# xmindflow/TransCeption

Hardware: AMD Instinct MI355X
Metric: images/sec fwd+bwd at 224x224 B=16 per GPU (higher is better)
Workload: dtype bf16; 1 GPU; TransCeption (MSTransception) 224x224 B=16/GPU fwd+bwd+SGD, synthetic Synapse npz slices via the device loader, name-seeded random-init weights; global_batch=16, image_size=224, parallelism=dp1, headline_mode=loader, headline_degraded=False, launch_mode=hipGraph replay

## Files before the change

transception_amd/build.py:

```python
from __future__ import annotations

import concurrent.futures as cf
import os
import subprocess
import sys

HERE = os.path.dirname(os.path.abspath(__file__))
CSRC = os.path.join(HERE, "csrc")
LIB = os.path.join(HERE, "libtransception_hip.so")
SOURCES = ["gemm.hip", "norm.hip", "dwconv.hip", "softmax.hip", "attention.hip", "attention_seg.hip", "elementwise.hip", "train.hip", "factoratt.hip", "data.hip", "mixffn.hip", "mixffn_bwd.hip", "effatt.hip", "cbam.hip", "ripm.hip", "linln.hip", "lncls.hip", "legacy.hip", "metrics.hip"]
FLAGS = ["--offload-arch=gfx950", "-O3", "-std=c++17", "-fPIC", "-ffp-contract=fast", "-munsafe-fp-atomics"]


def _hipcc() -> str:
    for c in (os.environ.get("HIPCC"), "/opt/rocm/bin/hipcc", "hipcc"):
        if c and (os.path.isabs(c) and os.path.exists(c) or not os.path.isabs(c)):
            return c
    raise RuntimeError("hipcc not found")


def _stale(target: str, deps) -> bool:
    if not os.path.exists(target):
        return True
    t = os.path.getmtime(target)
    return any(os.path.getmtime(d) > t for d in deps)


def build(force: bool = False, verbose: bool = True) -> str:
    hipcc = _hipcc()
    genv = {k: v for k, v in os.environ.items() if not k.startswith(("TC_ATTN_", "TC_AS_", "TC_DKV_", "TC_DQ_"))}
    for gen in ("gen_attn_asm.py", "gen_dkv_asm.py", "gen_dq_asm.py"):
        r = subprocess.run([sys.executable, os.path.join(CSRC, gen)], capture_output=True, text=True, env=genv)
        if r.returncode != 0:
            raise RuntimeError(f"{gen} failed:\n{r.stderr}")
    headers = [os.path.join(CSRC, "tc_common.h"), os.path.join(HERE, "..", "include", "transception_hip.h")]
    extra = {"attention_seg.hip": [os.path.join(CSRC, "attn_fwd_asm.inc"), os.path.join(CSRC, "attn_dkv_asm.inc"), os.path.join(CSRC, "attn_dq_asm.inc")]}
    objdir = os.path.join(HERE, "build")
    os.makedirs(objdir, exist_ok=True)
    jobs = []
    for src in SOURCES:
        s = os.path.join(CSRC, src)
        o = os.path.join(objdir, src.replace(".hip", ".o"))
        if force or _stale(o, [s] + headers + extra.get(src, [])):
            jobs.append((s, o))

    extra_flags = {"lncls.hip": ["-fno-slp-vectorize"]}

    def compile_one(job):
        s, o = job
        cmd = [hipcc, *FLAGS, *extra_flags.get(os.path.basename(s), []), "-c", s, "-o", o]
        r = subprocess.run(cmd, capture_output=True, text=True)
        if r.returncode != 0:
            raise RuntimeError(f"hipcc failed for {s}:\n{r.stderr}")
        return s

    with cf.ThreadPoolExecutor(max_workers=min(6, max(1, len(jobs)))) as ex:
        for s in ex.map(compile_one, jobs):
            if verbose:
                print(f"[build] compiled {os.path.basename(s)}")
    objs = [os.path.join(objdir, s.replace(".hip", ".o")) for s in SOURCES]
    if force or jobs or _stale(LIB, objs):
        r = subprocess.run([hipcc, "--offload-arch=gfx950", "-shared", "-fPIC", "-o", LIB, *objs], capture_output=True, text=True)
        if r.returncode != 0:
            raise RuntimeError(f"link failed:\n{r.stderr}")
        if verbose:
            print(f"[build] linked {LIB}")
    return LIB


if __name__ == "__main__":
    build(force="--force" in sys.argv)
```

transception_amd/csrc/effatt.hip:

```cpp
#include "tc_common.h"
#include <cstdlib>

namespace {

typedef float f32x16 __attribute__((ext_vector_type(16)));
typedef short s16x4_t __attribute__((ext_vector_type(4)));
typedef short s16x8_t __attribute__((ext_vector_type(8)));

constexpr int C = 64, PT = C + 8, TPW = 256, NW = 4, RT = 32 * NW, NRD = TPW / RT;
constexpr int TOUT = RT;
constexpr int F_M = 0, F_S = C, F_P = 2 * C, F_N = 2 * C + C * C;
constexpr int B1_DCTX = 0, B1_DWR = C * C, B1_DWQ = 2 * C * C, B1_DBR = 3 * C * C, B1_DBQ = B1_DBR + C, B1_N = B1_DBQ + C;
constexpr int B2_DWK = 0, B2_DWV = C * C, B2_DBK = 2 * C * C, B2_DBV = B2_DBK + C, B2_DG = B2_DBV + C, B2_DB = B2_DG + C, B2_N = B2_DB + C;
constexpr int SCW = 64 * 33;

struct EffDev {
    const void* t; const void* gamma; const void* beta;
    const void* wk; const void* bk; const void* wq; const void* bq; const void* wv; const void* bv; const void* wr; const void* br;
    void* out; float* ctx; float* kstat; float* part; float* dctx; float* rsum;
    const void* dout; void* dt; void* g1;
    int ldt, ldo, lddo, lddt, acc_dt, B, N, wpi;
    float eps;
};

template <typename V8> __device__ __forceinline__ V8 ld_tr(const bf16_t* lo, const bf16_t* hi) {
    const s16x4_t a = __builtin_amdgcn_ds_read_tr16_b64_v4i16((s16x4_t __attribute__((address_space(3)))*)(lo));
    const s16x4_t b = __builtin_amdgcn_ds_read_tr16_b64_v4i16((s16x4_t __attribute__((address_space(3)))*)(hi));
    return __builtin_bit_cast(V8, (s16x8_t)__builtin_shufflevector(a, b, 0, 1, 2, 3, 4, 5, 6, 7));
}
template <typename H> __device__ __forceinline__ void up8s(const uint4& r, float* o) {
    unpack2<H>(r.x, o[0], o[1]); unpack2<H>(r.y, o[2], o[3]); unpack2<H>(r.z, o[4], o[5]); unpack2<H>(r.w, o[6], o[7]);
}
struct Lane { int lane, l31, hh, gi, gq2, wv; };
__device__ __forceinline__ Lane lane_of() {
    Lane L; L.lane = threadIdx.x & 63; L.wv = threadIdx.x >> 6; L.l31 = L.lane & 31; L.hh = L.lane >> 5; L.gi = L.lane & 15; L.gq2 = (L.lane >> 4) & 1;
    return L;
}

__device__ __forceinline__ void zero2(f32x16 (&a)[2]) {
#pragma unroll
    for (int cb = 0; cb < 2; ++cb)
#pragma unroll
        for (int r = 0; r < 16; ++r) a[cb][r] = 0.f;
}
template <typename H> __device__ __forceinline__ void mm_w(const bf16_t* W, const bf16_t* X, const Lane& L, f32x16 (&acc)[2]) {
    using V8 = typename TcHalf<H>::v8;
#pragma unroll
    for (int kk = 0; kk < C / 16; ++kk) {
        const V8 xv = *reinterpret_cast<const V8*>(X + L.l31 * PT + kk * 16 + 8 * L.hh);
#pragma unroll
        for (int cb = 0; cb < 2; ++cb) acc[cb] = TcHalf<H>::mfma(*reinterpret_cast<const V8*>(W + (cb * 32 + L.l31) * PT + kk * 16 + 8 * L.hh), xv, acc[cb]);
    }
}
// ... 630 lines not shown
    if (!bwd) return f->out && !(f->ldo & 7) && !((uintptr_t)f->out & 15);
    if (!f->dout || !f->dt || !f->g1 || (f->lddo & 7) || (f->lddt & 7) || ((uintptr_t)f->dout & 15) || ((uintptr_t)f->dt & 15) || ((uintptr_t)f->g1 & 15)) return false;
    return f->dgamma && f->dbeta && f->dwk && f->dbk && f->dwq && f->dbq && f->dwv && f->dbv && f->dwr && f->dbr;
}
long long eff_scratch(int B, int N) {
    const long long nwv = (long long)B * ((N + TPW - 1) / TPW);
    const long long per = (B1_N + B2_N) > F_N ? (B1_N + B2_N) : F_N;
    return nwv * per + (long long)B * C * C + (long long)B * C;
}
EffDev eff_dev(const TcEffAtt* f) {
    EffDev p;
    p.t = f->t; p.gamma = f->gamma; p.beta = f->beta; p.wk = f->wk; p.bk = f->bk; p.wq = f->wq; p.bq = f->bq; p.wv = f->wv; p.bv = f->bv; p.wr = f->wr; p.br = f->br;
    p.out = f->out; p.ctx = f->ctx; p.kstat = f->kstat; p.part = f->part; p.dout = f->dout; p.dt = f->dt; p.g1 = f->g1;
    p.ldt = f->ldt; p.ldo = f->ldo; p.lddo = f->lddo; p.lddt = f->lddt; p.acc_dt = f->acc_dt; p.B = f->B; p.N = f->N; p.eps = f->eps;
    p.wpi = (f->N + TPW - 1) / TPW;
    const long long nwv = (long long)f->B * p.wpi;
    const long long per = (B1_N + B2_N) > F_N ? (B1_N + B2_N) : F_N;
    p.dctx = f->part + nwv * per;
    p.rsum = p.dctx + (long long)f->B * C * C;
    return p;
}

template <typename H> int eff_fwd(const TcEffAtt* f, hipStream_t s) {
    const EffDev p = eff_dev(f);
    const int nwv = f->B * p.wpi;
    hipLaunchKernelGGL((effatt_kv_kernel<H>), dim3(nwv), dim3(64 * NW), 0, s, p);
    if (tc_launch_status() != TC_OK) return TC_ERR_LAUNCH;
    hipLaunchKernelGGL(effatt_ctx_kernel, dim3(f->B, C), dim3(64), 0, s, p);
    if (tc_launch_status() != TC_OK) return TC_ERR_LAUNCH;
    hipLaunchKernelGGL((effatt_out_kernel<H>), dim3(f->B * ((f->N + TOUT - 1) / TOUT)), dim3(64 * NW), 0, s, p);
    return tc_launch_status();
}
template <typename H> int eff_bwd(const TcEffAtt* f, hipStream_t s) {
    const EffDev p = eff_dev(f);
    const int nwv = f->B * p.wpi;
    hipLaunchKernelGGL((effatt_bq_kernel<H>), dim3(nwv), dim3(64 * NW), 0, s, p);
    if (tc_launch_status() != TC_OK) return TC_ERR_LAUNCH;
    hipLaunchKernelGGL(effatt_dctx_kernel, dim3(f->B, C), dim3(64), 0, s, p);
    if (tc_launch_status() != TC_OK) return TC_ERR_LAUNCH;
    hipLaunchKernelGGL((effatt_bkv_kernel<H>), dim3(nwv), dim3(64 * NW), 0, s, p);
    if (tc_launch_status() != TC_OK) return TC_ERR_LAUNCH;
    FoldDev r;
    r.part = f->part; r.nwv = nwv; r.nper = B1_N + B2_N;
    float* dsts[12] = {nullptr, f->dwr, f->dwq, f->dbr, f->dbq, f->dwk, f->dwv, f->dbk, f->dbv, f->dgamma, f->dbeta, nullptr};
    const int offs[13] = {B1_DCTX, B1_DWR, B1_DWQ, B1_DBR, B1_DBQ, B1_N + B2_DWK, B1_N + B2_DWV, B1_N + B2_DBK, B1_N + B2_DBV, B1_N + B2_DG, B1_N + B2_DB, B1_N + B2_N, B1_N + B2_N};
    for (int i = 0; i < 12; ++i) r.dst[i] = dsts[i];
    for (int i = 0; i < 13; ++i) r.off[i] = offs[i];
    hipLaunchKernelGGL(effatt_fold_kernel, dim3((r.nper / 4 + 15) / 16), dim3(256), 0, s, r);
    return tc_launch_status();
}

}

extern "C" int tc_effatt_supported(int Cc, int dtype) { return Cc == C && (dtype == TC_BF16 || dtype == TC_F16); }
extern "C" long long tc_effatt_scratch_floats(int Cc, int B, int N) { return (Cc == C && B > 0 && N > 0) ? eff_scratch(B, N) : 0; }
extern "C" int tc_effatt_fwd(const TcEffAtt* f, int dtype, void* stream) {
    if (!eff_ok(f, false) || !tc_effatt_supported(f->C, dtype) || f->part_floats < eff_scratch(f->B, f->N)) return TC_ERR_ARG;
    return dtype == TC_BF16 ? eff_fwd<bf16_t>(f, (hipStream_t)stream) : eff_fwd<f16_t>(f, (hipStream_t)stream);
}
extern "C" int tc_effatt_bwd(const TcEffAtt* f, int dtype, void* stream) {
    if (!eff_ok(f, true) || !tc_effatt_supported(f->C, dtype) || f->part_floats < eff_scratch(f->B, f->N)) return TC_ERR_ARG;
    return dtype == TC_BF16 ? eff_bwd<bf16_t>(f, (hipStream_t)stream) : eff_bwd<f16_t>(f, (hipStream_t)stream);
}
```

transception_amd/engine.py:

```python
from __future__ import annotations

import ctypes as C
import os
from typing import Callable, Dict, List, Optional, Tuple

import torch

from ._lib import (ATTN_DKV_SPLITS, EW_COPY, EW_DEINTERLEAVE, EW_PATCHIFY, TcEffAtt, TcEwSeg, TcFfnBwd, TcFfnFused, ACT_COORD, ACT_GELU, ACT_HSWISH, ACT_NONE, ACT_SCALE, ACT_SIGMOID, FFN_EP, FFN_LN_A, FFN_LN_B, TC_BF16, TC_F16, TC_F32, TcDwFold, TcDwSeg, TcFfnSeg,
                   TcGemm, lib)

_DT = {torch.float32: TC_F32, torch.bfloat16: TC_BF16, torch.float16: TC_F16}

PROFILE: Optional[dict] = None


SEG_MARKS = os.environ.get("TC_SEG_MARKS", "")
SEG_LABELS: List[str] = []


def _timed(name: str, flops: float, fn):
    if PROFILE is None:
        fn()
        return
    e0, e1 = torch.cuda.Event(enable_timing=True), torch.cuda.Event(enable_timing=True)
# ... 790 lines not shown
                                   acc=1, splitk=self._splitk(t["C4"], t["Cin"], t["M"]), c_f32=1, nb1=Gn, sA=(t["M"] * t["C4"], 0),
                                   sB=(t["M"] * x.ld, 0), sC=(gs, 0), rowsum=_ptr(t["b1"].grad) if t["b1"].grad is not None else None, srow=gs,
                                   use_ws=False))
            self._launch_gemms(g2)
            for t in st:
                for k in ("gp", "part2", "dh"):
                    t.pop(k, None)
        self._rec(bwd)
        return [t["out"] for t in st_all]

    def _pass_grad_batched(self, v: Var, src: torch.Tensor, nb: int, M: int, N: int, sb_src: int, sb_dst: Optional[int] = None,
                           defer: bool = False):
        sb_dst = sb_src if sb_dst is None else sb_dst
        g, acc = self.wgrad(v, 0 if v.rows >= nb * M else (nb - 1) * sb_dst // v.root.cols)
        if defer:
            return TcEwSeg(EW_COPY, acc, src.data_ptr(), g.data_ptr(), sb_src, sb_dst, src.stride(0), g.stride(0), nb, M, N, 0, 0, 0)
        self.L.tc_copy3d(_ptr(src), sb_src, src.stride(0), _ptr(g), sb_dst, g.stride(0), nb, M, N, acc, self.dt, self.stream)

    def effatt_supported(self, t: Var, params: Optional[Tuple[P, ...]] = None) -> bool:
        if self.record and (not t.requires_grad or (params is not None and any(p.grad is None for p in params))):
            return False
        return (_EFFATT_FUSED and self.ngroups == 1 and self.dt != TC_F32
                and bool(self.L.tc_effatt_supported(t.cols, self.dt)) and t.data.is_contiguous())

    def eff_attention_block(self, t: Var, ln: Tuple[P, P], keys: Tuple[P, P], queries: Tuple[P, P], values: Tuple[P, P],
                            reproj: Tuple[P, P], B: int, N: int, eps: float = 1e-5) -> Var:
        L, Cc = self.L, t.cols
        assert t.rows == B * N and self.effatt_supported(t)
        out = self.new(t.rows, Cc)
        nf = int(L.tc_effatt_scratch_floats(Cc, B, N))
        ctx, kstat = self.f32(B, Cc, Cc), self.f32(B, 2, Cc)
        es = t.data.element_size()

        def desc(part, dout=None, dt=None, g1=None, acc=0, grads=False):
            f = TcEffAtt()
            f.t, f.gamma, f.beta = _ptr(t.data), _ptr(ln[0].data), _ptr(ln[1].data)
            for nm, (W, b) in (("k", keys), ("q", queries), ("v", values), ("r", reproj)):
                setattr(f, "w" + nm, _ptr(W.data)); setattr(f, "b" + nm, _ptr(b.data))
                if grads:
                    setattr(f, "dw" + nm, _ptr(W.grad)); setattr(f, "db" + nm, _ptr(b.grad))
            if grads:
                f.dgamma, f.dbeta = _ptr(ln[0].grad), _ptr(ln[1].grad)
            f.out, f.ctx, f.kstat, f.part, f.part_floats = _ptr(out.data), _ptr(ctx), _ptr(kstat), _ptr(part), nf
            f.ldt, f.ldo, f.C, f.B, f.N, f.eps = t.ld, out.ld, Cc, B, N, eps
            if dout is not None:
                f.dout, f.lddo, f.dt, f.lddt, f.g1, f.acc_dt = _ptr(dout), dout.stride(0), _ptr(dt), dt.stride(0), _ptr(g1), acc
            return f

        part = self.f32(nf)
        f = desc(part)
        self.n_launch += 3
        _timed("hbm:effatt_fwd (LayerNorm + EfficientAttention + residual: token statistics, context fold, output)",
               3.0 * t.rows * Cc * es, lambda: L.tc_effatt_fwd(C.byref(f), self.dt, self.stream))
        del part

        def bwd():
            dy = self.grad_of(out)
            if dy is None or not t.requires_grad:
                return
            gx, acc = self.wgrad(t)
            part = self.f32(nf)
            g1 = _empty((t.rows, Cc), self.dtype, self.dev)
            fb = desc(part, dy, gx, g1, acc, grads=True)
            self.n_launch += 4
            _timed("hbm:effatt_bwd (query side + d_ctx partials, d_ctx fold, key/value side + LayerNorm backward, parameter fold)",
                   (6.0 + acc) * t.rows * Cc * es, lambda: L.tc_effatt_bwd(C.byref(fb), self.dt, self.stream))
        self._rec(bwd)
        return out

    def layernorm(self, x: Var, g: P, b: P, eps: float = 1e-5, act: int = ACT_NONE, out: Optional[Var] = None,
                  stats: Optional[Tuple[torch.Tensor, torch.Tensor]] = None, launch: bool = True) -> Var:
        Gn = self.ngroups
        rows, Cc = x.rows // Gn, x.cols
        assert Gn == 1 or (g.gs > 0 and b.gs == g.gs)
        if out is None:
            out = self.new(x.rows, Cc)
        mean, rstd = stats if stats is not None else (self.f32(x.rows), self.f32(x.rows))
        es = x.data.element_size()
        if launch:
            _timed("hbm:layernorm_fwd", 2.0 * x.rows * Cc * es, lambda: self.L.tc_layernorm_fwd(
                _ptr(x.data), x.ld, _ptr(g.data), _ptr(b.data), _ptr(out.data), out.ld, _ptr(mean), _ptr(rstd), rows, Cc, eps, act, Gn, g.gs,
                self.dt, self.stream))

        def bwd():
            dy = self.grad_of(out)
            if dy is None or not x.requires_grad:
                return
            gx, acc = self.wgrad(x)
            fused = g.grad is not None
            nblk = int(self.L.tc_layernorm_bwd_nblk(rows, Cc)) if (fused and _LN_DEFER) else 0
            if nblk > 0:
                nf = Gn * nblk * 2 * Cc
                part = self.f32(nf)
                _timed("hbm:layernorm_bwd", (3.0 + acc) * x.rows * Cc * es, lambda: self.L.tc_layernorm_bwd_defer(
                    _ptr(dy), dy.stride(0), _ptr(x.data), x.ld, _ptr(g.data), _ptr(b.data), _ptr(mean), _ptr(rstd), _ptr(gx), gx.stride(0),
                    _ptr(gx) if acc else None, gx.stride(0), _ptr(g.grad), _ptr(b.grad), rows, Cc, act, Gn, g.gs, _ptr(part), nf, self.dt,
                    self.stream))
                self._ln_pending.append((part, g.grad, b.grad, g.gs, nblk, Cc, Gn))
                if len(self._ln_pending) == 64:
                    self._flush_param_folds()
                return
            if fused:
                ws = _workspace(self.dev)
                scratch, n = ws, ws.numel() // 4
                _timed("hbm:layernorm_bwd", (3.0 + acc) * x.rows * Cc * es, lambda: self.L.tc_layernorm_bwd(
                    _ptr(dy), dy.stride(0), _ptr(x.data), x.ld, _ptr(g.data), _ptr(b.data), _ptr(mean), _ptr(rstd), _ptr(gx), gx.stride(0),
                    _ptr(gx) if acc else None, gx.stride(0), _ptr(g.grad), _ptr(b.grad), rows, Cc, act, Gn, g.gs, _ptr(scratch), n, self.dt,
                    self.stream))
                return
            self.L.tc_layernorm_bwd(_ptr(dy), dy.stride(0), _ptr(x.data), x.ld, _ptr(g.data), _ptr(b.data), _ptr(mean),
                                    _ptr(rstd), _ptr(gx), gx.stride(0), _ptr(gx) if acc else None, gx.stride(0),
                                    None, None, rows, Cc, act, Gn, g.gs, None, 0, self.dt, self.stream)
        self._rec(bwd)
        return out
# ... 969 lines not shown
```

Measured before the change: 1463 images/sec.

## Add fused wide-channel EfficientAttention kernels for C=128 and C=320

Adds a new fused EfficientAttention path for channel widths 128 and 320. It uses three MFMA-based kernels for the forward pass (LayerNorm plus K/Q/V projections and token stats, context build, output) and a mix of fused kernels and grouped GEMMs for the backward pass. Before this, only C=64 had a fused path, so wider stages likely fell back to a sequence of generic ops. The forward now keeps its scratch buffer alive so the backward can reuse the saved intermediates (normalized input, k/q/v maps). The cost is more memory held between forward and backward, plus new code that could carry numerical or correctness risk.

```diff
diff --git a/transception_amd/build.py b/transception_amd/build.py
--- a/transception_amd/build.py
+++ b/transception_amd/build.py
@@ -8,7 +8,7 @@
 HERE = os.path.dirname(os.path.abspath(__file__))
 CSRC = os.path.join(HERE, "csrc")
 LIB = os.path.join(HERE, "libtransception_hip.so")
-SOURCES = ["gemm.hip", "norm.hip", "dwconv.hip", "softmax.hip", "attention.hip", "attention_seg.hip", "elementwise.hip", "train.hip", "factoratt.hip", "data.hip", "mixffn.hip", "mixffn_bwd.hip", "effatt.hip", "cbam.hip", "ripm.hip", "linln.hip", "lncls.hip", "legacy.hip", "metrics.hip"]
+SOURCES = ["gemm.hip", "norm.hip", "dwconv.hip", "softmax.hip", "attention.hip", "attention_seg.hip", "elementwise.hip", "train.hip", "factoratt.hip", "data.hip", "mixffn.hip", "mixffn_bwd.hip", "effatt.hip", "effatt_wide.hip", "cbam.hip", "ripm.hip", "linln.hip", "lncls.hip", "legacy.hip", "metrics.hip"]
 FLAGS = ["--offload-arch=gfx950", "-O3", "-std=c++17", "-fPIC", "-ffp-contract=fast", "-munsafe-fp-atomics"]
 
 
@@ -33,7 +33,7 @@
         r = subprocess.run([sys.executable, os.path.join(CSRC, gen)], capture_output=True, text=True, env=genv)
         if r.returncode != 0:
             raise RuntimeError(f"{gen} failed:\n{r.stderr}")
-    headers = [os.path.join(CSRC, "tc_common.h"), os.path.join(HERE, "..", "include", "transception_hip.h")]
+    headers = [os.path.join(CSRC, "tc_common.h"), os.path.join(CSRC, "effatt_wide.h"), os.path.join(HERE, "..", "include", "transception_hip.h")]
     extra = {"attention_seg.hip": [os.path.join(CSRC, "attn_fwd_asm.inc"), os.path.join(CSRC, "attn_dkv_asm.inc"), os.path.join(CSRC, "attn_dq_asm.inc")]}
     objdir = os.path.join(HERE, "build")
     os.makedirs(objdir, exist_ok=True)
diff --git a/transception_amd/csrc/effatt.hip b/transception_amd/csrc/effatt.hip
--- a/transception_amd/csrc/effatt.hip
+++ b/transception_amd/csrc/effatt.hip
@@ -1,4 +1,5 @@
 #include "tc_common.h"
+#include "effatt_wide.h"
 #include <cstdlib>
 
 namespace {
@@ -735,13 +736,18 @@
 
 }
 
-extern "C" int tc_effatt_supported(int Cc, int dtype) { return Cc == C && (dtype == TC_BF16 || dtype == TC_F16); }
-extern "C" long long tc_effatt_scratch_floats(int Cc, int B, int N) { return (Cc == C && B > 0 && N > 0) ? eff_scratch(B, N) : 0; }
+extern "C" int tc_effatt_supported(int Cc, int dtype) { return (Cc == C && (dtype == TC_BF16 || dtype == TC_F16)) || tcw::effatt_wide_supported(Cc, dtype); }
+extern "C" long long tc_effatt_scratch_floats(int Cc, int B, int N) {
+    if (Cc != C) return tcw::effatt_wide_scratch(Cc, B, N);
+    return (B > 0 && N > 0) ? eff_scratch(B, N) : 0;
+}
 extern "C" int tc_effatt_fwd(const TcEffAtt* f, int dtype, void* stream) {
+    if (f && f->C != C) return tcw::effatt_wide_fwd(f, dtype, stream);
     if (!eff_ok(f, false) || !tc_effatt_supported(f->C, dtype) || f->part_floats < eff_scratch(f->B, f->N)) return TC_ERR_ARG;
     return dtype == TC_BF16 ? eff_fwd<bf16_t>(f, (hipStream_t)stream) : eff_fwd<f16_t>(f, (hipStream_t)stream);
 }
 extern "C" int tc_effatt_bwd(const TcEffAtt* f, int dtype, void* stream) {
+    if (f && f->C != C) return tcw::effatt_wide_bwd(f, dtype, stream);
     if (!eff_ok(f, true) || !tc_effatt_supported(f->C, dtype) || f->part_floats < eff_scratch(f->B, f->N)) return TC_ERR_ARG;
     return dtype == TC_BF16 ? eff_bwd<bf16_t>(f, (hipStream_t)stream) : eff_bwd<f16_t>(f, (hipStream_t)stream);
 }
diff --git a/transception_amd/csrc/effatt_wide.h b/transception_amd/csrc/effatt_wide.h
--- /dev/null
+++ b/transception_amd/csrc/effatt_wide.h
@@ -0,0 +1,9 @@
+#pragma once
+#include "../../include/transception_hip.h"
+
+namespace tcw {
+__attribute__((visibility("hidden"))) int effatt_wide_supported(int C, int dtype);
+__attribute__((visibility("hidden"))) long long effatt_wide_scratch(int C, int B, int N);
+__attribute__((visibility("hidden"))) int effatt_wide_fwd(const TcEffAtt* f, int dtype, void* stream);
+__attribute__((visibility("hidden"))) int effatt_wide_bwd(const TcEffAtt* f, int dtype, void* stream);
+}
diff --git a/transception_amd/csrc/effatt_wide.hip b/transception_amd/csrc/effatt_wide.hip
--- /dev/null
+++ b/transception_amd/csrc/effatt_wide.hip
@@ -0,0 +1,632 @@
+#include "tc_common.h"
+#include "effatt_wide.h"
+
+namespace {
+
+typedef float f32x16 __attribute__((ext_vector_type(16)));
+typedef short s16x4_t __attribute__((ext_vector_type(4)));
+typedef short s16x8_t __attribute__((ext_vector_type(8)));
+
+constexpr int NW = 4, NT = 64 * NW, TT = 32;
+
+struct WideDev {
+    const void* t; const void* gamma; const void* beta;
+    const void* wk; const void* bk; const void* wq; const void* bq; const void* wv; const void* bv; const void* wr; const void* br;
+    void* out; float* ctx; float* kstat; const void* dout; void* dt;
+    float* dgamma; float* dbeta;
+    void* n1; void* km; void* qm; void* vm; void* am; void* dam; void* dkqv; void* ctx16;
+    float* tstat; float* dctx;
+    int ldt, ldo, lddo, lddt, acc_dt, B, N, tpi;
+    float eps;
+};
+
+template <typename V8> __device__ __forceinline__ V8 ld_tr(const bf16_t* lo, const bf16_t* hi) {
+    const s16x4_t a = __builtin_amdgcn_ds_read_tr16_b64_v4i16((s16x4_t __attribute__((address_space(3)))*)(lo));
+    const s16x4_t b = __builtin_amdgcn_ds_read_tr16_b64_v4i16((s16x4_t __attribute__((address_space(3)))*)(hi));
+    return __builtin_bit_cast(V8, (s16x8_t)__builtin_shufflevector(a, b, 0, 1, 2, 3, 4, 5, 6, 7));
+}
+template <typename H> __device__ __forceinline__ void up8(const uint4& r, float* o) {
+    unpack2<H>(r.x, o[0], o[1]); unpack2<H>(r.y, o[2], o[3]); unpack2<H>(r.z, o[4], o[5]); unpack2<H>(r.w, o[6], o[7]);
+}
+template <typename H> __device__ __forceinline__ uint4 pk8(const float* o) {
+    return make_uint4(pack2<H>(o[0], o[1]), pack2<H>(o[2], o[3]), pack2<H>(o[4], o[5]), pack2<H>(o[6], o[7]));
+}
+__device__ __forceinline__ void ldf8(const float* p, float* o) {
+    const float4 a = *reinterpret_cast<const float4*>(p), b = *reinterpret_cast<const float4*>(p + 4);
+    o[0] = a.x; o[1] = a.y; o[2] = a.z; o[3] = a.w; o[4] = b.x; o[5] = b.y; o[6] = b.z; o[7] = b.w;
+}
+template <typename H, typename WT> __device__ __forceinline__ uint4 ld8w(const WT* p) {
+    if constexpr (std::is_same<WT, float>::value) { float v[8]; ldf8(p, v); return pk8<H>(v); }
+    else return *reinterpret_cast<const uint4*>(p);
+}
+
+struct Lane { int lane, l31, hh, gi, gq2, wv; };
+__device__ __forceinline__ Lane lane_of() {
+    Lane L; L.lane = threadIdx.x & 63; L.wv = threadIdx.x >> 6; L.l31 = L.lane & 31; L.hh = L.lane >> 5; L.gi = L.lane & 15; L.gq2 = (L.lane >> 4) & 1;
+    return L;
+}
+
+template <int C, int SW> struct Geo {
+    static constexpr int PT = C + 8, PF = C + 4, PS = SW + 8;
+    static constexpr int SLAB = (SW * PT > C * PS) ? SW * PT : C * PS;
+};
+
+constexpr int slab_w(int C) { return C > 128 ? 64 : 128; }
+
+template <typename H, typename WT, int C, int SW, bool TR, bool ACC>
+__device__ __forceinline__ void tile_mm(const WT* __restrict__ W, const bf16_t* X, float* ft, bf16_t* slab, const Lane& L) {
+    using V8 = typename TcHalf<H>::v8;
+    using G = Geo<C, SW>;
+    constexpr int KSTEPS = SW == 128 ? C / 16 : C / 32;
+    const int blk = SW == 128 ? L.wv : (L.wv & 1), kh = SW == 128 ? 0 : (L.wv >> 1);
+    for (int o0 = 0; o0 < C; o0 += SW) {
+        const int nw = (C - o0) < SW ? (C - o0) : SW;
+        if (!TR) {
+            for (int i = threadIdx.x; i < nw * (C / 8); i += NT) {
+                const int r = i / (C / 8), cg = i - r * (C / 8);
+                *reinterpret_cast<uint4*>(slab + r * G::PT + cg * 8) = ld8w<H, WT>(W + (long long)(o0 + r) * C + cg * 8);
+            }
+        } else {
+            const int cpr = nw / 8;
+            for (int i = threadIdx.x; i < C * cpr; i += NT) {
+                const int r = i / cpr, cg = i - r * cpr;
+                *reinterpret_cast<uint4*>(slab + r * G::PS + cg * 8) = ld8w<H, WT>(W + (long long)r * C + o0 + cg * 8);
+            }
+        }
+        __syncthreads();
+        const bool act = blk * 32 < nw;
+        f32x16 acc;
+#pragma unroll
+        for (int r = 0; r < 16; ++r) acc[r] = 0.f;
+        if (act) {
+#pragma unroll 4
+            for (int ks = 0; ks < KSTEPS; ++ks) {
+                const int kk = kh * KSTEPS + ks;
+                const V8 xv = *reinterpret_cast<const V8*>(X + L.l31 * G::PT + kk * 16 + 8 * L.hh);
+                V8 a;
+                if (!TR) a = *reinterpret_cast<const V8*>(slab + (blk * 32 + L.l31) * G::PT + kk * 16 + 8 * L.hh);
+                else {
+                    const bf16_t* wp = slab + (16 * kk + 8 * L.hh + (L.gi >> 2)) * G::PS + blk * 32 + 16 * L.gq2 + 4 * (L.gi & 3);
+                    a = ld_tr<V8>(wp, wp + 4 * G::PS);
+                }
+                acc = TcHalf<H>::mfma(a, xv, acc);
+            }
+        }
+        float* fp = ft + L.l31 * G::PF + o0 + blk * 32 + 4 * L.hh;
+        if (SW == 128) {
+            if (act) {
+#pragma unroll
+                for (int gq = 0; gq < 4; ++gq) {
+                    float4 v = make_float4(acc[4 * gq], acc[4 * gq + 1], acc[4 * gq + 2], acc[4 * gq + 3]);
+                    if (ACC) { const float4 o = *reinterpret_cast<const float4*>(fp + 8 * gq); v.x += o.x; v.y += o.y; v.z += o.z; v.w += o.w; }
+                    *reinterpret_cast<float4*>(fp + 8 * gq) = v;
+                }
+            }
+        } else {
+#pragma unroll
+            for (int ph = 0; ph < 2; ++ph) {
+                if (act && kh == ph) {
+#pragma unroll
+                    for (int gq = 0; gq < 4; ++gq) {
+                        float4 v = make_float4(acc[4 * gq], acc[4 * gq + 1], acc[4 * gq + 2], acc[4 * gq + 3]);
+                        if (ACC || ph) { const float4 o = *reinterpret_cast<const float4*>(fp + 8 * gq); v.x += o.x; v.y += o.y; v.z += o.z; v.w += o.w; }
+                        *reinterpret_cast<float4*>(fp + 8 * gq) = v;
+                    }
+                }
+                if (ph == 0) __syncthreads();
+            }
+        }
+        __syncthreads();
+    }
+}
+
+template <typename H, int C> __device__ __forceinline__ void tile_load(bf16_t* X, const H* src, long long row0, int ld, int nv) {
+    for (int i = threadIdx.x; i < TT * (C / 8); i += NT) {
+        const int r = i / (C / 8), cg = i - r * (C / 8);
+        *reinterpret_cast<uint4*>(X + r * (C + 8) + cg * 8) = r < nv ? *reinterpret_cast<const uint4*>(src + (row0 + r) * ld + cg * 8) : make_uint4(0u, 0u, 0u, 0u);
+    }
+}
+template <typename H, int C> __device__ __forceinline__ void tile_store(const bf16_t* X, H* dst, long long row0, int ld, int nv) {
+    for (int i = threadIdx.x; i < TT * (C / 8); i += NT) {
+        const int r = i / (C / 8), cg = i - r * (C / 8);
+        if (r < nv) *reinterpret_cast<uint4*>(dst + (row0 + r) * ld + cg * 8) = *reinterpret_cast<const uint4*>(X + r * (C + 8) + cg * 8);
+    }
+}
+template <typename H, int C> __device__ __forceinline__ void load_vec(float* v, const void* src) {
+    for (int i = threadIdx.x; i < C; i += NT) v[i] = ldf<H>(reinterpret_cast<const H*>(src) + i);
+}
+template <typename H, int C> __device__ __forceinline__ void row_stats(const bf16_t* X, int r, int q, float eps, float& mean, float& rstd) {
+    float s = 0.f;
+#pragma unroll
+    for (int j = 0; j < C / 64; ++j) {
+        float v[8];
+        up8<H>(*reinterpret_cast<const uint4*>(X + r * (C + 8) + (q + 8 * j) * 8), v);
+#pragma unroll
+        for (int e = 0; e < 8; ++e) s += v[e];
+    }
+    mean = tc_group_sum<8>(s) * (1.0f / C);
+    float q2 = 0.f;
+#pragma unroll
+    for (int j = 0; j < C / 64; ++j) {
+        float v[8];
+        up8<H>(*reinterpret_cast<const uint4*>(X + r * (C + 8) + (q + 8 * j) * 8), v);
+#pragma unroll
+        for (int e = 0; e < 8; ++e) { const float d = v[e] - mean; q2 += d * d; }
+    }
+    rstd = rsqrtf(tc_group_sum<8>(q2) * (1.0f / C) + eps);
+}
+
+struct Where { int b, w; long long row0; int nv; };
+__device__ __forceinline__ Where where_am_i(int tpi, int N) {
+    Where q;
+    q.b = blockIdx.x / tpi; q.w = blockIdx.x - q.b * tpi;
+    q.row0 = (long long)q.b * N + (long long)q.w * TT;
+    q.nv = min(TT, N - q.w * TT);
+    return q;
+}
+
+template <typename H, int C>
+__global__ __launch_bounds__(NT) void wide_kqv_kernel(const WideDev p) {
+    using G = Geo<C, slab_w(C)>;
+    constexpr int PT = G::PT, PF = G::PF;
+    __shared__ __attribute__((aligned(16))) bf16_t xt[TT * PT], yt[TT * PT], slab[G::SLAB];
+    __shared__ __attribute__((aligned(16))) float ft[TT * PF];
+    __shared__ float gam[C], bet[C], bia[C];
+    const Lane L = lane_of();
+    const Where w = where_am_i(p.tpi, p.N);
+    const int r = threadIdx.x >> 3, q = threadIdx.x & 7;
+    tile_load<H, C>(xt, reinterpret_cast<const H*>(p.t), w.row0, p.ldt, w.nv);
+    load_vec<H, C>(gam, p.gamma); load_vec<H, C>(bet, p.beta); load_vec<H, C>(bia, p.bk);
+    __syncthreads();
+    {
+        float mean, rstd;
+        row_stats<H, C>(xt, r, q, p.eps, mean, rstd);
+#pragma unroll
+        for (int j = 0; j < C / 64; ++j) {
+            const int c0 = (q + 8 * j) * 8;
+            float v[8];
+            up8<H>(*reinterpret_cast<const uint4*>(xt + r * PT + c0), v);
+#pragma unroll
+            for (int e = 0; e < 8; ++e) v[e] = (v[e] - mean) * rstd * gam[c0 + e] + bet[c0 + e];
+            *reinterpret_cast<uint4*>(xt + r * PT + c0) = pk8<H>(v);
+        }
+    }
+    __syncthreads();
+    tile_store<H, C>(xt, reinterpret_cast<H*>(p.n1), w.row0, C, w.nv);
+    tile_mm<H, H, C, slab_w(C), false, false>(reinterpret_cast<const H*>(p.wk), xt, ft, slab, L);
+#pragma unroll
+    for (int j = 0; j < C / 64; ++j) {
+        const int c0 = (q + 8 * j) * 8;
+        float v[8];
+        ldf8(ft + r * PF + c0, v);
+#pragma unroll
+        for (int e = 0; e < 8; ++e) v[e] += bia[c0 + e];
+        *reinterpret_cast<uint4*>(yt + r * PT + c0) = pk8<H>(v);
+    }
+    __syncthreads();
+    tile_store<H, C>(yt, reinterpret_cast<H*>(p.km), w.row0, C, w.nv);
+    for (int c = threadIdx.x; c < C; c += NT) {
+        float m = -3.0e38f;
+        for (int rr = 0; rr < w.nv; ++rr) m = fmaxf(m, ldf<H>(reinterpret_cast<const H*>(yt) + rr * PT + c));
+        float s = 0.f;
+        for (int rr = 0; rr < w.nv; ++rr) s += __expf(ldf<H>(reinterpret_cast<const H*>(yt) + rr * PT + c) - m);
+        float* ts = p.tstat + (long long)blockIdx.x * 2 * C;
+        ts[c] = m; ts[C + c] = s;
+    }
+    __syncthreads();
+    load_vec<H, C>(bia, p.bq);
+    tile_mm<H, H, C, slab_w(C), false, false>(reinterpret_cast<const H*>(p.wq), xt, ft, slab, L);
+    {
+        float v[C / 64][8], m = -3.0e38f, s = 0.f;
+#pragma unroll
+        for (int j = 0; j < C / 64; ++j) {
+            const int c0 = (q + 8 * j) * 8;
+            ldf8(ft + r * PF + c0, v[j]);
+#pragma unroll
+            for (int e = 0; e < 8; ++e) { v[j][e] += bia[c0 + e]; m = fmaxf(m, v[j][e]); }
+        }
+        m = tc_group_max<8>(m);
+#pragma unroll
+        for (int j = 0; j < C / 64; ++j)
+#pragma unroll
+            for (int e = 0; e < 8; ++e) { v[j][e] = __expf(v[j][e] - m); s += v[j][e]; }
+        const float inv = 1.0f / tc_group_sum<8>(s);
+#pragma unroll
+        for (int j = 0; j < C / 64; ++j) {
+#pragma unroll
+            for (int e = 0; e < 8; ++e) v[j][e] *= inv;
+            *reinterpret_cast<uint4*>(yt + r * PT + (q + 8 * j) * 8) = pk8<H>(v[j]);
+        }
+    }
+    __syncthreads();
+    tile_store<H, C>(yt, reinterpret_cast<H*>(p.qm), w.row0, C, w.nv);
+    load_vec<H, C>(bia, p.bv);
+    tile_mm<H, H, C, slab_w(C), false, false>(reinterpret_cast<const H*>(p.wv), xt, ft, slab, L);
+#pragma unroll
+    for (int j = 0; j < C / 64; ++j) {
+        const int c0 = (q + 8 * j) * 8;
+        float v[8];
+        ldf8(ft + r * PF + c0, v);
+#pragma unroll
+        for (int e = 0; e < 8; ++e) v[e] += bia[c0 + e];
+        if (r < w.nv) *reinterpret_cast<uint4*>(reinterpret_cast<H*>(p.vm) + (w.row0 + r) * C + c0) = pk8<H>(v);
+    }
+}
+
+constexpr int CP = 40;
+template <typename H, int C>
+__global__ __launch_bounds__(NT) void wide_ctx_kernel(const WideDev p) {
+    using V8 = typename TcHalf<H>::v8;
+    __shared__ __attribute__((aligned(16))) bf16_t et[NW][64 * CP], vt[NW][64 * CP];
+    __shared__ float red[NW][32 * 33], mz[2][32];
+    const Lane L = lane_of();
+    const int jb = blockIdx.x, ib = blockIdx.y, b = blockIdx.z;
+    if (threadIdx.x < 32) {
+        const int c = ib * 32 + threadIdx.x;
+        const float* ts = p.tstat + (long long)b * p.tpi * 2 * C;
+        float M = -3.0e38f;
+        for (int t = 0; t < p.tpi; ++t) M = fmaxf(M, ts[(long long)t * 2 * C + c]);
+        float Z = 0.f;
+        for (int t = 0; t < p.tpi; ++t) Z += __expf(ts[(long long)t * 2 * C + c] - M) * ts[(long long)t * 2 * C + C + c];
+        mz[0][threadIdx.x] = M; mz[1][threadIdx.x] = 1.0f / Z;
+        if (jb == 0) { p.kstat[(long long)b * 2 * C + c] = M; p.kstat[(long long)b * 2 * C + C + c] = Z; }
+    }
+    __syncthreads();
+    const H* K = reinterpret_cast<const H*>(p.km) + (long long)b * p.N * C + ib * 32;
+    const H* V = reinterpret_cast<const H*>(p.vm) + (long long)b * p.N * C + jb * 32;
+    bf16_t* E = et[L.wv]; bf16_t* VV = vt[L.wv];
+    f32x16 acc;
+#pragma unroll
+    for (int r = 0; r < 16; ++r) acc[r] = 0.f;
+    const int col = 16 * L.gq2 + 4 * (L.gi & 3);
+    for (int tok0 = L.wv * 64; tok0 < p.N; tok0 += NW * 64) {
+        uint4 kv[4], vv[4];
+#pragma unroll
+        for (int j = 0; j < 4; ++j) {
+            const int i = L.lane + 64 * j, r = i >> 2, cg = i & 3;
+            const bool ok = tok0 + r < p.N;
+            kv[j] = ok ? *reinterpret_cast<const uint4*>(K + (long long)(tok0 + r) * C + cg * 8) : make_uint4(0u, 0u, 0u, 0u);
+            vv[j] = ok ? *reinterpret_cast<const uint4*>(V + (long long)(tok0 + r) * C + cg * 8) : make_uint4(0u, 0u, 0u, 0u);
+        }
+#pragma unroll
+        for (int j = 0; j < 4; ++j) {
+            const int i = L.lane + 64 * j, r = i >> 2, cg = i & 3;
+            const bool ok = tok0 + r < p.N;
+            float k[8];
+            up8<H>(kv[j], k);
+#pragma unroll
+            for (int e = 0; e < 8; ++e) k[e] = ok ? __expf(k[e] - mz[0][cg * 8 + e]) : 0.f;
+            *reinterpret_cast<uint4*>(E + r * CP + cg * 8) = pk8<H>(k);
+            *reinterpret_cast<uint4*>(VV + r * CP + cg * 8) = vv[j];
+        }
+        __builtin_amdgcn_fence(__ATOMIC_RELEASE, "wavefront"); __builtin_amdgcn_wave_barrier();
+#pragma unroll
+        for (int ks = 0; ks < 4; ++ks) {
+            const int row = 16 * ks + 8 * L.hh + (L.gi >> 2);
+            const V8 a = ld_tr<V8>(E + row * CP + col, E + (row + 4) * CP + col);
+            const V8 bb = ld_tr<V8>(VV + row * CP + col, VV + (row + 4) * CP + col);
+            acc = TcHalf<H>::mfma(a, bb, acc);
+        }
+        __builtin_amdgcn_fence(__ATOMIC_RELEASE, "wavefront"); __builtin_amdgcn_wave_barrier();
+    }
+#pragma unroll
+    for (int r = 0; r < 16; ++r) red[L.wv][((r & 3) + 8 * (r >> 2) + 4 * L.hh) * 33 + L.l31] = acc[r];
+    __syncthreads();
+    for (int e = threadIdx.x; e < 32 * 32; e += NT) {
+        const int i = e >> 5, j = e & 31;
+        const float v = (red[0][i * 33 + j] + red[1][i * 33 + j] + red[2][i * 33 + j] + red[3][i * 33 + j]) * mz[1][i];
+        const long long o = ((long long)b * C + ib * 32 + i) * C + jb * 32 + j;
+        p.ctx[o] = v;
+        stf<H>(reinterpret_cast<H*>(p.ctx16) + o, v);
+    }
+}
+
+template <typename H, int C>
+__global__ __launch_bounds__(NT) void wide_out_kernel(const WideDev p) {
+    using G = Geo<C, slab_w(C)>;
+    constexpr int PT = G::PT, PF = G::PF;
+    __shared__ __attribute__((aligned(16))) bf16_t xt[TT * PT], yt[TT * PT], slab[G::SLAB];
+    __shared__ __attribute__((aligned(16))) float ft[TT * PF];
+    __shared__ float bia[C];
+    const Lane L = lane_of();
+    const Where w = where_am_i(p.tpi, p.N);
+    const int r = threadIdx.x >> 3, q = threadIdx.x & 7;
+    tile_load<H, C>(xt, reinterpret_cast<const H*>(p.qm), w.row0, C, w.nv);
+    load_vec<H, C>(bia, p.br);
+    tile_mm<H, H, C, slab_w(C), true, false>(reinterpret_cast<const H*>(p.ctx16) + (long long)w.b * C * C, xt, ft, slab, L);
+#pragma unroll
+    for (int j = 0; j < C / 64; ++j) {
+        const int c0 = (q + 8 * j) * 8;
+        float v[8];
+        ldf8(ft + r * PF + c0, v);
+        const uint4 pk = pk8<H>(v);
+        *reinterpret_cast<uint4*>(yt + r * PT + c0) = pk;
+        if (r < w.nv) *reinterpret_cast<uint4*>(reinterpret_cast<H*>(p.am) + (w.row0 + r) * C + c0) = pk;
+    }
+    tile_mm<H, H, C, slab_w(C), false, false>(reinterpret_cast<const H*>(p.wr), yt, ft, slab, L);
+    if (r < w.nv) {
+#pragma unroll
+        for (int j = 0; j < C / 64; ++j) {
+            const int c0 = (q + 8 * j) * 8;
+            float v[8], x[8];
+            ldf8(ft + r * PF + c0, v);
+            up8<H>(*reinterpret_cast<const uint4*>(reinterpret_cast<const H*>(p.t) + (w.row0 + r) * p.ldt + c0), x);
+#pragma unroll
+            for (int e = 0; e < 8; ++e) v[e] += bia[c0 + e] + x[e];
+            *reinterpret_cast<uint4*>(reinterpret_cast<H*>(p.out) + (w.row0 + r) * p.ldo + c0) = pk8<H>(v);
+        }
+    }
+}
+
+template <typename H, int C>
+__global__ __launch_bounds__(NT) void wide_bq_kernel(const WideDev p) {
+    using G = Geo<C, slab_w(C)>;
+    constexpr int PT = G::PT, PF = G::PF;
+    __shared__ __attribute__((aligned(16))) bf16_t xt[TT * PT], yt[TT * PT], slab[G::SLAB];
+    __shared__ __attribute__((aligned(16))) float ft[TT * PF];
+    const Lane L = lane_of();
+    const Where w = where_am_i(p.tpi, p.N);
+    const int r = threadIdx.x >> 3, q = threadIdx.x & 7;
+    tile_load<H, C>(xt, reinterpret_cast<const H*>(p.dout), w.row0, p.lddo, w.nv);
+    tile_mm<H, H, C, slab_w(C), true, false>(reinterpret_cast<const H*>(p.wr), xt, ft, slab, L);
+#pragma unroll
+    for (int j = 0; j < C / 64; ++j) {
+        const int c0 = (q + 8 * j) * 8;
+        float v[8];
+        ldf8(ft + r * PF + c0, v);
+        const uint4 pk = pk8<H>(v);
+        *reinterpret_cast<uint4*>(yt + r * PT + c0) = pk;
+        if (r < w.nv) *reinterpret_cast<uint4*>(reinterpret_cast<H*>(p.dam) + (w.row0 + r) * C + c0) = pk;
+    }
+    tile_mm<H, H, C, slab_w(C), false, false>(reinterpret_cast<const H*>(p.ctx16) + (long long)w.b * C * C, yt, ft, slab, L);
+    {
+        float qs[C / 64][8], g[C / 64][8], dot = 0.f;
+#pragma unroll
+        for (int j = 0; j < C / 64; ++j) {
+            const int c0 = (q + 8 * j) * 8;
+            ldf8(ft + r * PF + c0, g[j]);
+            const uint4 qv = r < w.nv ? *reinterpret_cast<const uint4*>(reinterpret_cast<const H*>(p.qm) + (w.row0 + r) * C + c0) : make_uint4(0u, 0u, 0u, 0u);
+            up8<H>(qv, qs[j]);
+#pragma unroll
+            for (int e = 0; e < 8; ++e) dot += qs[j][e] * g[j][e];
+        }
+        dot = tc_group_sum<8>(dot);
+        if (r < w.nv) {
+#pragma unroll
+            for (int j = 0; j < C / 64; ++j) {
+#pragma unroll
+                for (int e = 0; e < 8; ++e) g[j][e] = qs[j][e] * (g[j][e] - dot);
+                *reinterpret_cast<uint4*>(reinterpret_cast<H*>(p.dkqv) + (w.row0 + r) * (3 * C) + C + (q + 8 * j) * 8) = pk8<H>(g[j]);
+            }
+        }
+    }
+}
+
+template <typename H, int C>
+__global__ __launch_bounds__(NT) void wide_bkv_kernel(const WideDev p) {
+    constexpr int SW = slab_w(C);
+    using G = Geo<C, SW>;
+    constexpr int PT = G::PT, PF = G::PF;
+    __shared__ __attribute__((aligned(16))) bf16_t st[TT * PT], yt[TT * PT], zt[TT * PT], slab[G::SLAB];
+    __shared__ __attribute__((aligned(16))) float ft[TT * PF];
+    __shared__ float gam[C], km[C], kiz[C], rs[C], rst[TT][2];
+    const Lane L = lane_of();
+    const Where w = where_am_i(p.tpi, p.N);
+    const int r = threadIdx.x >> 3, q = threadIdx.x & 7;
+    const float* DC = p.dctx + (long long)w.b * C * C;
+    const H* KM = reinterpret_cast<const H*>(p.km);
+    H* DKQV = reinterpret_cast<H*>(p.dkqv);
+    load_vec<H, C>(gam, p.gamma);
+    for (int i = threadIdx.x; i < C; i += NT) { km[i] = p.kstat[(long long)w.b * 2 * C + i]; kiz[i] = 1.0f / p.kstat[(long long)w.b * 2 * C + C + i]; }
+    {
+        const float* CX = p.ctx + (long long)w.b * C * C;
+        for (int i = 0; i < C / 32; ++i) {
+            const int c = r + 32 * i;
+            float s = 0.f;
+#pragma unroll
+            for (int j = 0; j < C / 64; ++j) {
+                float a[8], bb[8];
+                ldf8(DC + c * C + (q + 8 * j) * 8, a); ldf8(CX + c * C + (q + 8 * j) * 8, bb);
+                up8<H>(pk8<H>(a), a);
+#pragma unroll
+                for (int e = 0; e < 8; ++e) s += a[e] * bb[e];
+            }
+            s = tc_group_sum<8>(s);
+            if (q == 0) rs[c] = s;
+        }
+    }
+    __syncthreads();
+#pragma unroll
+    for (int j = 0; j < C / 64; ++j) {
+        const int c0 = (q + 8 * j) * 8;
+        float k[8];
+        up8<H>(r < w.nv ? *reinterpret_cast<const uint4*>(KM + (w.row0 + r) * C + c0) : make_uint4(0u, 0u, 0u, 0u), k);
+#pragma unroll
+        for (int e = 0; e < 8; ++e) k[e] = r < w.nv ? __expf(k[e] - km[c0 + e]) * kiz[c0 + e] : 0.f;
+        *reinterpret_cast<uint4*>(st + r * PT + c0) = pk8<H>(k);
+    }
+    tile_mm<H, float, C, SW, true, false>(DC, st, ft, slab, L);
+#pragma unroll
+    for (int j = 0; j < C / 64; ++j) {
+        const int c0 = (q + 8 * j) * 8;
+        float v[8];
+        ldf8(ft + r * PF + c0, v);
+        const uint4 pk = pk8<H>(v);
+        *reinterpret_cast<uint4*>(yt + r * PT + c0) = pk;
+        if (r < w.nv) *reinterpret_cast<uint4*>(DKQV + (w.row0 + r) * (3 * C) + 2 * C + c0) = pk;
+    }
+    tile_load<H, C>(st, reinterpret_cast<const H*>(p.vm), w.row0, C, w.nv);
+    tile_mm<H, float, C, SW, false, false>(DC, st, ft, slab, L);
+#pragma unroll
+    for (int j = 0; j < C / 64; ++j) {
+        const int c0 = (q + 8 * j) * 8;
+        float v[8], k[8];
+        ldf8(ft + r * PF + c0, v);
+        up8<H>(r < w.nv ? *reinterpret_cast<const uint4*>(KM + (w.row0 + r) * C + c0) : make_uint4(0u, 0u, 0u, 0u), k);
+#pragma unroll
+        for (int e = 0; e < 8; ++e) v[e] = r < w.nv ? __expf(k[e] - km[c0 + e]) * kiz[c0 + e] * (v[e] - rs[c0 + e]) : 0.f;
+        const uint4 pk = pk8<H>(v);
+        *reinterpret_cast<uint4*>(zt + r * PT + c0) = pk;
+        if (r < w.nv) *reinterpret_cast<uint4*>(DKQV + (w.row0 + r) * (3 * C) + c0) = pk;
+    }
+    tile_load<H, C>(st, reinterpret_cast<const H*>(DKQV) + C, w.row0, 3 * C, w.nv);
+    tile_mm<H, H, C, SW, true, false>(reinterpret_cast<const H*>(p.wk), zt, ft, slab, L);
+    tile_mm<H, H, C, SW, true, true>(reinterpret_cast<const H*>(p.wv), yt, ft, slab, L);
+    tile_mm<H, H, C, SW, true, true>(reinterpret_cast<const H*>(p.wq), st, ft, slab, L);
+    tile_load<H, C>(st, reinterpret_cast<const H*>(p.t), w.row0, p.ldt, w.nv);
+    __syncthreads();
+    {
+        float mean, rstd;
+        row_stats<H, C>(st, r, q, p.eps, mean, rstd);
+        if (q == 0) { rst[r][0] = mean; rst[r][1] = rstd; }
+        float dg[C / 64][8], xh[C / 64][8], s1 = 0.f, s2 = 0.f;
+#pragma unroll
+        for (int j = 0; j < C / 64; ++j) {
+            const int c0 = (q + 8 * j) * 8;
+            float x[8];
+            ldf8(ft + r * PF + c0, dg[j]);
+            up8<H>(*reinterpret_cast<const uint4*>(st + r * PT + c0), x);
+#pragma unroll
+            for (int e = 0; e < 8; ++e) {
+                xh[j][e] = (x[e] - mean) * rstd;
+                dg[j][e] = r < w.nv ? dg[j][e] * gam[c0 + e] : 0.f;
+                s1 += dg[j][e]; s2 += dg[j][e] * xh[j][e];
+            }
+        }
+        const float k1 = tc_group_sum<8>(s1) * (1.0f / C), k2 = tc_group_sum<8>(s2) * (1.0f / C);
+        if (r < w.nv) {
+#pragma unroll
+            for (int j = 0; j < C / 64; ++j) {
+                const int c0 = (q + 8 * j) * 8;
+                float o[8], y[8];
+                up8<H>(*reinterpret_cast<const uint4*>(reinterpret_cast<const H*>(p.dout) + (w.row0 + r) * p.lddo + c0), y);
+#pragma unroll
+                for (int e = 0; e < 8; ++e) o[e] = rstd * (dg[j][e] - k1 - xh[j][e] * k2);
+                up8<H>(pk8<H>(o), o);
+#pragma unroll
+                for (int e = 0; e < 8; ++e) o[e] += y[e];
+                H* dp = reinterpret_cast<H*>(p.dt) + (w.row0 + r) * p.lddt + c0;
+                if (p.acc_dt) {
+                    up8<H>(*reinterpret_cast<const uint4*>(dp), y);
+#pragma unroll
+                    for (int e = 0; e < 8; ++e) o[e] += y[e];
+                }
+                *reinterpret_cast<uint4*>(dp) = pk8<H>(o);
+            }
+        }
+    }
+    __syncthreads();
+    for (int c = threadIdx.x; c < C; c += NT) {
+        float sg = 0.f, sb = 0.f;
+        for (int rr = 0; rr < w.nv; ++rr) {
+            const float d = ft[rr * PF + c];
+            const float xhat = (ldf<H>(reinterpret_cast<const H*>(st) + rr * PT + c) - rst[rr][0]) * rst[rr][1];
+            sg += d * xhat; sb += d;
+        }
+        atomicAdd(p.dgamma + c, sg); atomicAdd(p.dbeta + c, sb);
+    }
+}
+
+bool wide_width(int C) { return C == 128 || C == 320; }
+long long al4(long long n) { return (n + 3) & ~3LL; }
+int tiles_per_image(int N) { return (N + TT - 1) / TT; }
+
+bool wide_ok(const TcEffAtt* f, bool bwd) {
+    if (!f || !f->t || !f->gamma || !f->beta || !f->wk || !f->bk || !f->wq || !f->bq || !f->wv || !f->bv || !f->wr || !f->br || !f->ctx || !f->kstat || !f->part) return false;
+    if (!wide_width(f->C) || f->B < 1 || f->N < 1 || f->B > 65535 || (f->ldt & 7) || ((uintptr_t)f->t & 15) || ((uintptr_t)f->part & 15) || ((uintptr_t)f->ctx & 15)) return false;
+    if (((uintptr_t)f->wk | (uintptr_t)f->wq | (uintptr_t)f->wv | (uintptr_t)f->wr) & 15) return false;
+    if ((long long)f->B * f->N >= 0x7fffffffLL / (f->ldt > 3 * f->C ? f->ldt : 3 * f->C)) return false;
+    if (!bwd) return f->out && !(f->ldo & 7) && !((uintptr_t)f->out & 15);
+    if (!f->dout || !f->dt || (f->lddo & 7) || (f->lddt & 7) || ((uintptr_t)f->dout & 15) || ((uintptr_t)f->dt & 15)) return false;
+    return f->dgamma && f->dbeta && f->dwk && f->dbk && f->dwq && f->dbq && f->dwv && f->dbv && f->dwr && f->dbr;
+}
+
+WideDev wide_dev(const TcEffAtt* f, int esz) {
+    WideDev p;
+    p.t = f->t; p.gamma = f->gamma; p.beta = f->beta; p.wk = f->wk; p.bk = f->bk; p.wq = f->wq; p.bq = f->bq; p.wv = f->wv; p.bv = f->bv; p.wr = f->wr; p.br = f->br;
+    p.out = f->out; p.ctx = f->ctx; p.kstat = f->kstat; p.dout = f->dout; p.dt = f->dt; p.dgamma = f->dgamma; p.dbeta = f->dbeta;
+    p.ldt = f->ldt; p.ldo = f->ldo; p.lddo = f->lddo; p.lddt = f->lddt; p.acc_dt = f->acc_dt; p.B = f->B; p.N = f->N; p.eps = f->eps;
+    p.tpi = tiles_per_image(f->N);
+    (void)esz;
+    const long long C = f->C, rows = (long long)f->B * f->N, map = al4(rows * C / 2);
+    float* s = f->part;
+    p.n1 = s; s += map; p.km = s; s += map; p.qm = s; s += map; p.vm = s; s += map; p.am = s; s += map; p.dam = s; s += map;
+    p.dkqv = s; s += 3 * map;
+    p.ctx16 = s; s += al4(f->B * C * C / 2);
+    p.dctx = s; s += (long long)f->B * C * C;
+    p.tstat = s;
+    return p;
+}
+
+int wgrad_split(int C, long long rows) {
+    const long long tiles = (long long)((C + 63) / 64) * ((C + 63) / 64);
+    long long sk = 512 / tiles;
+    if (sk > rows / 384) sk = rows / 384;
+    if (sk > 128) sk = 128;
+    return sk < 1 ? 1 : (int)sk;
+}
+TcGemm wgrad_desc(const void* dy, int lddy, const void* x, int ldx, float* dw, float* db, int C, long long rows, int dtype) {
+    TcGemm g = {};
+    g.A = dy; g.B = x; g.C = dw; g.M = C; g.N = C; g.K = (int)rows; g.lda = lddy; g.ldb = ldx; g.ldc = C;
+    g.transA = 1; g.transB = 0; g.nb1 = 1; g.nb2 = 1; g.alpha = 1.0f; g.accumulate = 1; g.act = TC_ACT_NONE;
+    g.splitk = wgrad_split(C, rows); g.dtype = dtype; g.c_f32 = 1; g.rowsum = db;
+    return g;
+}
+
+template <typename H, int C> int wide_fwd_t(const TcEffAtt* f, hipStream_t s) {
+    const WideDev p = wide_dev(f, 2);
+    const int ntile = f->B * p.tpi;
+    hipLaunchKernelGGL((wide_kqv_kernel<H, C>), dim3(ntile), dim3(NT), 0, s, p);
+    if (tc_launch_status() != TC_OK) return TC_ERR_LAUNCH;
+    hipLaunchKernelGGL((wide_ctx_kernel<H, C>), dim3(C / 32, C / 32, f->B), dim3(NT), 0, s, p);
+    if (tc_launch_status() != TC_OK) return TC_ERR_LAUNCH;
+    hipLaunchKernelGGL((wide_out_kernel<H, C>), dim3(ntile), dim3(NT), 0, s, p);
+    return tc_launch_status();
+}
+template <typename H, int C> int wide_bwd_t(const TcEffAtt* f, int dtype, hipStream_t s) {
+    const WideDev p = wide_dev(f, 2);
+    const int ntile = f->B * p.tpi;
+    const long long rows = (long long)f->B * f->N;
+    hipLaunchKernelGGL((wide_bq_kernel<H, C>), dim3(ntile), dim3(NT), 0, s, p);
+    if (tc_launch_status() != TC_OK) return TC_ERR_LAUNCH;
+    TcGemm g[3];
+    g[0] = TcGemm{};
+    g[0].A = p.qm; g[0].B = p.dam; g[0].C = p.dctx; g[0].M = C; g[0].N = C; g[0].K = f->N; g[0].lda = C; g[0].ldb = C; g[0].ldc = C;
+    g[0].transA = 1; g[0].transB = 0; g[0].nb1 = f->B; g[0].nb2 = 1; g[0].sA1 = (long long)f->N * C; g[0].sB1 = (long long)f->N * C; g[0].sC1 = (long long)C * C;
+    g[0].alpha = 1.0f; g[0].splitk = 1; g[0].dtype = dtype; g[0].c_f32 = 1;
+    g[1] = wgrad_desc(f->dout, f->lddo, p.am, C, f->dwr, f->dbr, C, rows, dtype);
+    int rc = tc_gemm_multi(g, 2, s);
+    if (rc != TC_OK) return rc;
+    hipLaunchKernelGGL((wide_bkv_kernel<H, C>), dim3(ntile), dim3(NT), 0, s, p);
+    if (tc_launch_status() != TC_OK) return TC_ERR_LAUNCH;
+    const H* d3 = reinterpret_cast<const H*>(p.dkqv);
+    g[0] = wgrad_desc(d3, 3 * C, p.n1, C, f->dwk, f->dbk, C, rows, dtype);
+    g[1] = wgrad_desc(d3 + C, 3 * C, p.n1, C, f->dwq, f->dbq, C, rows, dtype);
+    g[2] = wgrad_desc(d3 + 2 * C, 3 * C, p.n1, C, f->dwv, f->dbv, C, rows, dtype);
+    return tc_gemm_multi(g, 3, s);
+}
+
+}
+
+namespace tcw {
+
+int effatt_wide_supported(int C, int dtype) { return wide_width(C) && (dtype == TC_BF16 || dtype == TC_F16); }
+long long effatt_wide_scratch(int C, int B, int N) {
+    if (!wide_width(C) || B < 1 || N < 1) return 0;
+    const long long rows = (long long)B * N, map = al4(rows * C / 2);
+    return 9 * map + al4((long long)B * C * C / 2) + (long long)B * C * C + (long long)B * tiles_per_image(N) * 2 * C;
+}
+int effatt_wide_fwd(const TcEffAtt* f, int dtype, void* stream) {
+    if (!wide_ok(f, false) || !effatt_wide_supported(f->C, dtype) || f->part_floats < effatt_wide_scratch(f->C, f->B, f->N)) return TC_ERR_ARG;
+    hipStream_t s = (hipStream_t)stream;
+    if (f->C == 128) return dtype == TC_BF16 ? wide_fwd_t<bf16_t, 128>(f, s) : wide_fwd_t<f16_t, 128>(f, s);
+    return dtype == TC_BF16 ? wide_fwd_t<bf16_t, 320>(f, s) : wide_fwd_t<f16_t, 320>(f, s);
+}
+int effatt_wide_bwd(const TcEffAtt* f, int dtype, void* stream) {
+    if (!wide_ok(f, true) || !effatt_wide_supported(f->C, dtype) || f->part_floats < effatt_wide_scratch(f->C, f->B, f->N)) return TC_ERR_ARG;
+    hipStream_t s = (hipStream_t)stream;
+    if (f->C == 128) return dtype == TC_BF16 ? wide_bwd_t<bf16_t, 128>(f, dtype, s) : wide_bwd_t<f16_t, 128>(f, dtype, s);
+    return dtype == TC_BF16 ? wide_bwd_t<bf16_t, 320>(f, dtype, s) : wide_bwd_t<f16_t, 320>(f, dtype, s);
+}
+
+}
diff --git a/transception_amd/engine.py b/transception_amd/engine.py
--- a/transception_amd/engine.py
+++ b/transception_amd/engine.py
@@ -866,14 +866,12 @@
         self.n_launch += 3
         _timed("hbm:effatt_fwd (LayerNorm + EfficientAttention + residual: token statistics, context fold, output)",
                3.0 * t.rows * Cc * es, lambda: L.tc_effatt_fwd(C.byref(f), self.dt, self.stream))
-        del part
 
         def bwd():
             dy = self.grad_of(out)
             if dy is None or not t.requires_grad:
                 return
             gx, acc = self.wgrad(t)
-            part = self.f32(nf)
             g1 = _empty((t.rows, Cc), self.dtype, self.dev)
             fb = desc(part, dy, gx, g1, acc, grads=True)
             self.n_launch += 4
```

Result: slower. 1419 images/sec (-3.0%).
